# PhilipPragerUrbina/DOGERAY

Measured on AMD Instinct MI355X. Metric: Mrays/sec + ms/frame, 1M-tri .rts at 1920x1080, higher is better.
Workload: dtype f32

## Files before the change

### dogeray_amd/csrc/context.cpp

```cpp
#include <climits>
#include <exception>

#include "context.hpp"
#include "linearise.hpp"

using namespace dr;

namespace {

constexpr int ANY = INT_MIN;
struct Option { const char* name; int dr_context::*member; int lo, hi; unsigned only; bool reorders; };
const Option OPTIONS[] = {
    {"kernel", &dr_context::kernel, DR_KERNEL_TILE, DR_KERNEL_PERSISTENT, 0, false},
    {"occupancy", &dr_context::occupancy, 4, 6, 0, false},
    {"schedule", &dr_context::schedule, 0, 2, 0, false},
    {"heavy_factor", &dr_context::heavy_factor, -1, 1000, 0, true},
    {"coop_steps", &dr_context::coop_steps, 0, INT_MAX, 0, false},
    {"coop_lanes", &dr_context::coop_lanes, 1, 64, 0, false},
    {"split_parts", &dr_context::split_parts, 1, 8, 1u << 1 | 1u << 2 | 1u << 4 | 1u << 8, false},
    {"split_waves", &dr_context::split_waves, 1, 1000, 0, true},
    {"split_steps", &dr_context::split_steps, 16, 4080, 0, true},
    {"short_one_queue", &dr_context::short_one_queue, ANY, 0, 0, true},
    {"coop_rounds", &dr_context::coop_rounds, 1, 16, 0, false},
    {"reserve_cus", &dr_context::reserve_cus, 0, 64, 0, false},
    {"wave_log", &dr_context::wave_log_on, 0, 1, 0, false},
    {"coop_tiles_per_wave", &dr_context::coop_tiles_per_wave, 0, INT_MAX, 0, false},
    {"pipe_streams", &dr_context::pipe_streams, 2, dr_context::PIPE_STREAMS, 0, false},
    {"pipe_lean", &dr_context::pipe_lean, ANY, 0, 0, false},
    {"pipe_group", &dr_context::pipe_group, 1, dr_context::PIPE_GROUP_MAX, 0, false},
    {"xcd_regions", &dr_context::xcd_regions, ANY, 0, 0, true},
    {"batch_frames", &dr_context::batch_frames, 1, 256, 0, false},
    {"feedback", &dr_context::feedback, ANY, 0, 0, true},
    {"order_follows_camera", &dr_context::order_follows_camera, ANY, 0, 0, false},
    {"feedback_every", &dr_context::feedback_every, 1, INT_MAX, 0, false},
    {"wide_tree", &dr_context::wide_tree, 0, 2, 0, false},
    {"denoise_tiles", &dr_context::denoise_tiles, 0, 1, 0, false},
    {"moments", &dr_context::moments_opt, 0, 1, 0, false},
    {"denoise_variance", &dr_context::denoise_variance, 0, 1, 0, false},
    {"camera_cert", &dr_context::camera_cert, 0, 1, 0, false},
    {"cert_factor", &dr_context::cert_factor, 1, 10000, 0, false},
    {"cert_levels",  &dr_context::cert_levels, 0, 1, 0, false},
    {"camera_entry",  &dr_context::camera_entry, 0, 1, 0, false},
    {"sky_tiles",  &dr_context::sky_tiles, 0, 2, 0, false},
    {"trace_kernel",  &dr_context::trace_kernel, 0, 2, 0, false},
    {"radiance_kernel",  &dr_context::radiance_kernel, 0, 2, 0, false},
    {"allhits_kernel",  &dr_context::allhits_kernel, 0, 2, 0, false},
};

const Option* find_option(const std::string& name) {
  for (const Option& o : OPTIONS) if (name == o.name) return &o;
  return nullptr;
}

int flush_held(dr_context* c) {
  if (c->pipe_pending.empty()) return DR_OK;
  HIP_TRY(hipSetDevice(c->device));
  return pipeline_flush(c);
}

int set_option(dr_context* c, const std::string& name, int v) {
  const Option* o = find_option(name);
  if (!o) { set_error("unknown option '" + name + "'"); return DR_ERR_INVALID; }
  if (o->lo == ANY) v = v != 0;
  else if (v < o->lo || v > o->hi || (o->only && !(o->only >> v & 1u))) { set_error("value not supported for option '" + name + "'"); return DR_ERR_INVALID; }
  DR_TRY(flush_held(c));
  if (name == "split_steps") v &= ~15;
  else if (name == "wave_log") {
    if (v && !c->wave_log) {
      if (hipSetDevice(c->device) != hipSuccess || c->wave_log.alloc((size_t)WAVE_LOG_WAVES * 16) != DR_OK) { set_error("cannot allocate the wave log"); return DR_ERR_DEVICE; }
      (void)hipMemsetAsync(c->wave_log, 0, c->wave_log.n * sizeof(unsigned long long), c->stream);
    }
  }
  else if (name == "pipe_streams") {
    if (v != c->pipe_streams) {
      if (hipSetDevice(c->device) != hipSuccess || join_pipeline(c) != DR_OK || hipStreamSynchronize(c->stream) != hipSuccess) { set_error("pipe_streams: cannot drain the pipeline"); return DR_ERR_DEVICE; }
      for (int k = 0; k < dr_context::PIPE_DEPTH; k++) { c->pipe_slot[k].drained = true; c->pipe_slot[k].count = 0; c->pipe_slot[k].unwaited = 0; }
      c->pipe_parked.clear();
      c->pipe_next = 0; c->pipe_groups = 0;
    }
  }
  else if (name == "camera_cert" || name == "cert_factor" || o->member == &dr_context::cert_levels || o->member == &dr_context::camera_entry ||
           o->member == &dr_context::sky_tiles) c->cert_valid = false;
  c->*(o->member) = v;
  if (o->reorders) c->order_valid = false;
  return DR_OK;
}

}

dr_context::~dr_context() {
  (void)hipSetDevice(device);
  if (stream) (void)hipStreamSynchronize(stream);
  for (int k = 1; k < PIPE_STREAMS; k++) if (pipe_stream[k]) (void)hipStreamSynchronize(pipe_stream[k]);
  if (acc_stream) (void)hipStreamSynchronize(acc_stream);
  if (ev0) (void)hipEventDestroy(ev0);
  if (ev1) (void)hipEventDestroy(ev1);
  for (int k = 0; k < 2; k++) { if (pev0[k]) (void)hipEventDestroy(pev0[k]); if (pev1[k]) (void)hipEventDestroy(pev1[k]); }
  for (PipeSlot& sl : pipe_slot) {
    if (sl.rendered) (void)hipEventDestroy(sl.rendered);
// ... 298 lines not shown
```

### dogeray_amd/csrc/context.hpp

```cpp
#pragma once
#include <hip/hip_runtime_api.h>

#include <cmath>
#include <cstring>
#include <map>
#include <string>
#include <vector>

#include "kernels.hpp"
#include "params_host.hpp"
#include "scene_host.hpp"

#define HIP_TRY(expr)                                                                      \
  do {                                                                                     \
    hipError_t e_ = (expr);                                                                \
    if (e_ != hipSuccess) {                                                                \
      dr::set_error(std::string(#expr) + ": " + hipGetErrorString(e_));                    \
      return DR_ERR_DEVICE;                                                                \
    }                                                                                      \
  } while (0)

#define DR_TRY(expr)                                                                       \
  do {                                                                                     \
    const int rc_ = (expr);                                                                \
// ... 4 lines not shown

template <class T, bool PINNED = false>
struct DevMem {
  T* p = nullptr;
  size_t n = 0;
  DevMem() = default;
  DevMem(const DevMem&) = delete;
  DevMem& operator=(const DevMem&) = delete;
  ~DevMem() { release(); }
  operator T*() const { return p; }
  void release() {
    if (p) (void)(PINNED ? hipHostFree(p) : hipFree(p));
    p = nullptr; n = 0;
  }
  void swap(DevMem& o) { std::swap(p, o.p); std::swap(n, o.n); }
  int grow(size_t need, hipStream_t stream) {
    if (p && n >= need) return DR_OK;
    if (p) { HIP_TRY(hipStreamSynchronize(stream)); release(); }
    const hipError_t e = PINNED ? hipHostMalloc((void**)&p, need * sizeof(T), hipHostMallocDefault) : hipMalloc((void**)&p, need * sizeof(T));
    if (e != hipSuccess) { p = nullptr; set_error(std::string("cannot allocate ") + std::to_string(need * sizeof(T)) + " bytes: " + hipGetErrorString(e)); return DR_ERR_DEVICE; }
    n = need;
    return DR_OK;
  }
  int alloc(size_t count) { release(); return grow(count ? count : 1, nullptr); }
  int upload(const std::vector<T>& src) { DR_TRY(alloc(src.size())); return put(src.data(), src.size()); }
  int put(const T* src, size_t count) { if (count) HIP_TRY(hipMemcpy(p, src, count * sizeof(T), hipMemcpyHostToDevice)); return DR_OK; }
  int get(T* dst, size_t count) const { if (count) HIP_TRY(hipMemcpy(dst, p, count * sizeof(T), hipMemcpyDeviceToHost)); return DR_OK; }
};

struct GuideKey {
  bool valid = false;
  float st[13] = {0};
  int W = 0, H = 0;
  uint64_t gen = 0;
  bool matches(const float* settings13, int w, int h, uint64_t scene_gen) const {
    return valid && W == w && H == h && gen == scene_gen && memcmp(st, settings13, sizeof(st)) == 0;
  }
  void store(const float* settings13, int w, int h, uint64_t scene_gen) {
    memcpy(st, settings13, sizeof(st));
    W = w; H = h; gen = scene_gen; valid = true;
  }
};

struct LaunchSite {
  hipStream_t stream;
  bool hold_order;
  bool lean;
};

constexpr int TILE_COUNTERS = 1024;
constexpr int LAUNCH_COUNTERS = MAX_REGIONS + 1;

}

struct dr_context {
  template <class T> using DevMem = dr::DevMem<T>;
  int device = 0;
  hipStream_t stream = nullptr;
  hipEvent_t ev0 = nullptr, ev1 = nullptr;
  hipEvent_t pev0[2] = {nullptr, nullptr}, pev1[2] = {nullptr, nullptr};
  bool pending[2] = {false, false}; uint64_t pending_frames[2] = {0, 0}, pending_samples[2] = {0, 0}; int pending_next = 0;
  DevMem<dr::DevUnit> walk; size_t walk_bytes = 0;
  DevMem<dr::DevUnit> wide; size_t wide_bytes = 0; int wide_depth = 0, wide_nodes = 0; float wide_pmax = 0; dr::WideMu wide_mu = {0, 0, 0}; int wide_own_bounds = 0;
  int wide_tree = 2;
  DevMem<dr::DevPair> pairs;
  DevMem<dr::DevPrim> prims;
  DevMem<dr::DevShade> shade;
  DevMem<dr::DevTex> tex;
  DevMem<uint32_t> texels;
  int n_prims = 0, n_tex = 0, tree_depth = 0;
  std::vector<int> slot_to_orig;
  DevMem<int32_t> slot_to_orig_dev;
  DevMem<uint8_t> aov_staging;
  DevMem<uint8_t> query_staging;
  DevMem<uint32_t> query_scratch;
  DevMem<unsigned> query_cursor;
  int trace_kernel = 0, radiance_kernel = 0, allhits_kernel = 0;
  float near_lmax = 0;
  DevMem<float> dn_planes;
  dr::GuideKey dn_key;
  DevMem<uint8_t> dn_staging;
  DevMem<float> up_planes;
  dr::GuideKey up_key;
  int up_passes = 0;
  uint64_t scene_gen = 0;
  DevMem<int32_t> accum2;
  DevMem<int32_t> hist_buf[2];
  int32_t* hist = nullptr; int hist_cur = 0;
  DevMem<float> rp_planes[2];
  dr::GuideKey rp_key; int rp_cur = 0;
  DevMem<unsigned long long> rp_counts;
  int rp_passes = 0;
  int moments_opt = 0;
  int denoise_variance = 0;
  DevMem<unsigned long long> m2_buf[2];
  unsigned long long* m2 = nullptr; int m2_cur = 0;
  DevMem<unsigned long long> err_counts;
  DevMem<float> err_staging;
  int denoise_tiles = 1;
  int camera_cert = 1;
  int cert_factor = 40;
  int cert_levels = 1;
  DevMem<uint32_t> cert_mask;
  DevMem<uint32_t> cert_level;
  bool cert_valid = false;
  bool cert_ok = false;
  bool entry_ok = false;
  float cert_key[22] = {0};
  float cert_seen[22] = {0};
  float cert_k[dr::CERT_MAX_LEVELS + 1] = {1};
  int cert_tiles = 0;
  int camera_entry = 1;
  DevMem<uint32_t> wide_leaf_rec, wide_range;
  int wide_leaves = 0;
  DevMem<uint32_t> entry_mm;
  DevMem<uint32_t> cert_word;
  int sky_tiles = 2;
  DevMem<int> launch_order, launch_region_start, sky_list;
  DevMem<unsigned> sky_counts;
  bool sky_split_last = false;
  uint64_t cert_gen = 0;
  uint64_t order_gen = 0;
  uint64_t sky_key[5] = {0, 0, 0, 0, 0}; bool sky_key_valid = false;
  DevMem<int32_t> frame;
  DevMem<int32_t> accum; int accW = 0, accH = 0;
  DevMem<uint8_t> present;
  DevMem<int32_t> packed[2];
  DevMem<unsigned long long> counters;
  DevMem<unsigned> tile_counters; int tile_cursor = 0; int num_cus = 256;
  DevMem<unsigned> pixel_cost, tile_cost; DevMem<int> tile_order, region_start;
  int order_capacity = 0;
  bool order_valid = false;
  int order_age = 0;
  int order_follows_camera = 1;
  int feedback_every = 8;
  float order_key[18] = {0};
  int order_args[5] = {0, 0, 0, 0, 0};
  int feedback = 1;
  int stripe_mod = 1, stripe_rem = 0;
  int traversal = DR_TRAVERSAL_WIDE;
  int count = 0;
  int kernel = DR_KERNEL_PERSISTENT;
  int occupancy = 6;
  int schedule = 0;
  int xcd_regions = 1;
  int heavy_factor = 1;
  int coop_steps = 2;
  int coop_tiles_per_wave = 32;
  int coop_lanes = 8;
  int split_parts = 4;
  int split_waves = 12;
  int split_steps = 400;
  int short_one_queue = 1;
  int coop_rounds = 2;
  int reserve_cus = 0;
  int wave_log_on = 0;
  DevMem<unsigned long long> wave_log; int wave_log_waves = 0;
  int batch_frames = 32;
  float cur_settings[13] = {0};
  dr_stats stats;
  static constexpr int PIPE_STREAMS = 4;
  static constexpr int PIPE_DEPTH = PIPE_STREAMS + 1;
  int pipe_streams = 2;
  int pipe_lean = 0;
  hipStream_t pipe_stream[PIPE_STREAMS] = {nullptr, nullptr, nullptr, nullptr}, acc_stream = nullptr;
  static constexpr int PIPE_GROUP_MAX = 16;
  struct PipeSlot {
    DevMem<int32_t> frames; size_t elems_each = 0; int cap_frames = 0;
    int rect[6] = {-1, 0, 0, 0, 0, 0};
// ... 56 lines not shown
```

### dogeray_amd/csrc/context_render.cpp

```cpp
#include "context.hpp"

namespace dr {

void fill_scene(const dr_context* c, RenderParams& P) {
  P.walk = c->walk; P.walk_bytes = (uint32_t)c->walk_bytes; P.pairs = c->pairs; P.prims = c->prims; P.shade = c->shade; P.tex = c->tex; P.texels = c->texels;
  P.wide = c->wide; P.wide_bytes = (uint32_t)c->wide_bytes; P.wide_pmax = c->wide_pmax; P.wide_mu = c->wide_mu;
}

static int tiles_per_wave(const dr_context* c, const LaunchSite& site) {
  return site.lean ? 0 : c->coop_tiles_per_wave;
}

int make_params(dr_context* c, const LaunchSite& site, const float* st, int W, int H, float background, uint64_t seed, RenderParams& P, int batch_hint) {
  if (!c->walk) { set_error("no scene uploaded"); return DR_ERR_INVALID; }
  memset(&P, 0, sizeof(P));
  if (const char* why = fill_view_params(st, W, H, background, seed, c->stripe_mod, c->stripe_rem, P)) { set_error(why); return DR_ERR_INVALID; }
  if (P.backtex >= c->n_tex) { set_error("backtex refers to a texture that is not loaded"); return DR_ERR_INVALID; }
  memcpy(c->cur_settings, st, sizeof(c->cur_settings));
  fill_scene(c, P);
  P.counters = c->counters;
  P.wave_log = c->wave_log_on ? c->wave_log.p : nullptr;
  P.coop_steps = c->coop_steps; P.coop_rounds = c->coop_rounds; P.split_parts = c->split_parts;
  P.coop_lanes = c->coop_lanes;
  const int tiles = P.ncols * P.gy;
// ... 51 lines not shown
    c->cert_valid = false;
    c->cert_ok = c->entry_ok = false;
    c->cert_gen++;
    if (fill_cert_view(P, a_star, want_cert ? c->wide_mu.e : 1.0f, cv)) {
      if (c->cert_level.grow(cert_level_words(tiles), site.stream) != DR_OK || c->cert_word.grow((size_t)tiles, site.stream) != DR_OK ||
          (want_entry && c->entry_mm.grow(entry_mm_words(tiles), site.stream) != DR_OK)) return;
      for (float& k : c->cert_k) k = 1.0f;
      if (want_cert) {
        cert_ladder(c->cert_factor, c->cert_levels != 0, cv);
        if (c->cert_mask.grow(cert_mask_words(tiles, cv.n_levels), site.stream) != DR_OK) return;
        launch_cert_mask(site.stream, c->prims, c->n_prims, cv, c->cert_mask, c->cert_level, tiles);
        for (int g = 1; g <= CERT_MAX_LEVELS; g++) c->cert_k[g] = g <= cv.n_levels ? cert_factor_k(cv.level_a[g - 1]) : 1.0f;
      } else {
        (void)hipMemsetAsync(c->cert_level, 0, cert_level_words(tiles) * sizeof(uint32_t), site.stream);
      }
      launch_camera_entry(site.stream, c->wide, c->wide_leaf_rec, c->wide_range, c->wide_leaves, cv, want_entry ? c->entry_mm.p : nullptr, c->cert_level, c->cert_word, tiles);
      c->cert_ok = want_cert; c->entry_ok = want_entry;
    }
    memcpy(c->cert_key, key, sizeof(key));
    c->cert_tiles = tiles;
    c->cert_valid = true;
  }
  if (c->cert_ok || c->entry_ok) { P.cert_level = c->cert_word; memcpy(P.wide_cert_k, c->cert_k, sizeof(P.wide_cert_k)); }
}

bool sky_split(dr_context* c, const LaunchSite& site, RenderParams& P, int tiles, const int*& order, const int*& region_start, unsigned* pcost, unsigned* cursor) {
  if (!c->sky_tiles || !c->entry_ok || !P.cert_level || site.hold_order || site.stream != c->stream || P.out_frame_stride != 0) return false;
  if (P.max_depth <= 0 || !(P.spp_f > 0.0f)) return false;
  if (!plan_sky_split(plan_persistent(persistent_cfg(c, site), (long long)tiles * P.batch, P.coop_steps, false, P.wave_log != nullptr))) return false;
  const uint64_t key[5] = {c->cert_gen, order ? 1u : 0u, order ? c->order_gen : 0u, (uint64_t)tiles, (uint64_t)P.regions};
  const bool room = c->launch_order.n >= (size_t)tiles && c->sky_list.n >= (size_t)tiles && c->launch_region_start.p && c->sky_counts.p;
  if (!(room && c->sky_key_valid && memcmp(c->sky_key, key, sizeof(key)) == 0)) {
    c->sky_key_valid = false;
    if (c->launch_order.grow((size_t)tiles, site.stream) != DR_OK || c->sky_list.grow((size_t)tiles, site.stream) != DR_OK ||
        c->launch_region_start.grow(2 * MAX_REGIONS + 1, site.stream) != DR_OK || c->sky_counts.grow(2, site.stream) != DR_OK)
      return false;
    launch_sky_split(site.stream, order, region_start, P.region_start, P.cert_level, tiles, P.regions, c->launch_order, c->launch_region_start, c->sky_list, c->sky_counts);
    memcpy(c->sky_key, key, sizeof(key));
    c->sky_key_valid = true;
  }
  if (c->sky_tiles == 2) {
    P.sky_list = c->sky_list; P.sky_counts = c->sky_counts; P.sky_cursor = cursor;
    P.sky_chunk = sky_chunk_frames(P.batch, P.accumulate == 2 ? SKY_CHUNK : 0);
  } else launch_sky_tiles(site.stream, P, c->sky_list, c->sky_counts, pcost);
  order = c->launch_order; region_start = c->launch_region_start;
  return true;
}

}

int enqueue_frame(dr_context* c, const LaunchSite& site, const RenderParams& P_in) {
  RenderParams P = P_in;
  const int tiles = P.ncols * P.gy;
  if (uses_persistent(c)) {
    if (c->tile_cursor + LAUNCH_COUNTERS > TILE_COUNTERS) {
      (void)hipMemsetAsync(c->tile_counters, 0, TILE_COUNTERS * sizeof(unsigned), site.stream);
      c->tile_cursor = 0;
    }
    unsigned* counter = c->tile_counters + c->tile_cursor;
    c->tile_cursor += LAUNCH_COUNTERS;
    const int* order; unsigned* pcost;
    if (site.hold_order) {
      float geom[5];
      order_geometry(P, geom);
      order = (c->order_valid && c->order_capacity >= tiles && memcmp(c->order_key + 13, geom, sizeof(geom)) == 0) ? c->tile_order.p : nullptr;
      pcost = nullptr;
    } else feedback_buffers(c, site, P, tiles, order, pcost);
    if (!c->wave_log_on) P.wave_log = nullptr;
    cert_prepare(c, site, P, tiles);
    const int* launch_order = order; const int* launch_rstart = c->region_start;
    c->sky_split_last = sky_split(c, site, P, tiles, launch_order, launch_rstart, pcost, counter + MAX_REGIONS);
    const int log_waves = launch_persistent_kernel(site.stream, P, persistent_cfg(c, site), counter, launch_order, launch_rstart, pcost);
    if (log_waves < 0) { set_error("the persistent kernel has no build for this launch (launch_plan.hpp)"); return DR_ERR_DEVICE; }
    c->wave_log_waves = log_waves;
    if (pcost && !order) c->order_age = 0;
    if (pcost && (c->order_age < 2 || c->order_age % c->feedback_every == 0)) {
      const int split_limit = plan_split_limit(c->num_cus, c->occupancy, c->split_parts, c->split_waves);
      launch_tile_feedback(site.stream, c->pixel_cost, c->tile_cost, c->tile_order, c->region_start, tiles, P.regions, c->heavy_factor, c->split_steps, split_limit);
      c->order_gen++;
      c->order_args[0] = tiles; c->order_args[1] = P.regions; c->order_args[2] = c->heavy_factor; c->order_args[3] = c->split_steps; c->order_args[4] = split_limit;
      c->order_valid = true;
    }
    c->order_age++;
    return DR_OK;
  }
  c->sky_split_last = false;
  launch_tile_kernel(site.stream, P, traversal_of(c), c->count != 0, c->occupancy);
  return DR_OK;
}

}

using namespace dr;

namespace {

int launch_render(dr_context* c, const RenderParams& P) {
  int tiles = P.ncols * P.gy;
  if (tiles <= 0) return DR_OK;
  HIP_TRY(hipEventRecord(c->ev0, c->stream));
  DR_TRY(enqueue_frame(c, c->own_site(), P));
  HIP_TRY(hipGetLastError());
  HIP_TRY(hipEventRecord(c->ev1, c->stream));
  return DR_OK;
}

// ... 114 lines not shown
```

### dogeray_amd/csrc/device_layout.h

```cpp
#pragma once
#include <stdint.h>

namespace dr {

struct DevUnit {
  float f[4];
};
constexpr int WALK_UNITS_INTERNAL = 2;
constexpr int WALK_UNITS_LEAF = 4;
constexpr int WALK_SLOT_BITS = 26;
constexpr int WALK_KIND_SPHERE = 0, WALK_KIND_TRIANGLE = 1, WALK_KIND_NONE = 2;

inline uint32_t wide_node_first_child(const uint32_t* w) { return w[3] & 0xffffffu; }
inline uint32_t wide_node_valid(const uint32_t* w) { return (w[3] >> 24) & 15u; }
inline uint32_t wide_node_leaf_mask(const uint32_t* w) { return w[3] >> 28; }
inline uint32_t wide_node_lo(const uint32_t* w, int axis) { return w[4 + axis]; }
inline uint32_t wide_node_hi(const uint32_t* w, int axis) { return w[7 + axis]; }
inline uint32_t wide_node_scale24_bits(const uint32_t* w, int axis) { return axis == 0 ? w[10] << 16 : (axis == 1 ? w[10] & 0xffff0000u : w[11]); }
struct WideMu {
  float e;
  float l;
  float v;
};
struct CertView {
// ... 68 lines not shown
static_assert(CERT_MAX_LEVELS < (1 << ENTRY_SHIFT), "a grade fits under the entry code");
static_assert(sizeof(DevUnit) == 16, "DevUnit");
static_assert(sizeof(DevPair) == 64, "DevPair");
static_assert(sizeof(DevPrim) == 48, "DevPrim");
static_assert(sizeof(DevShade) == 128, "DevShade");
static_assert(sizeof(DevTex) == 16, "DevTex");

struct RenderParams {
  const DevUnit* walk;
  uint32_t walk_bytes;
  uint32_t pad_;
  const DevUnit* wide;
  uint32_t wide_bytes;
  float wide_pmax;
  const DevPair* pairs;
  const DevPrim* prims;
  const DevShade* shade;
  const DevTex* tex;
  const uint32_t* texels;
  int32_t* out;
  unsigned long long* counters;
  unsigned long long* wave_log;
  float from[3], llc[3], hor[3], ver[3], uu[3], vu[3];
  float lens_radius;
  float bgint;
  float scale;
  float spp_f;
  double den_w, den_h;
  uint64_t seed;
  int32_t W, H;
  int32_t gx, gy;
  int32_t ncols;
  int32_t stripe_mod, stripe_rem;
  uint32_t seed_stride;
  int32_t max_depth;
  int32_t backtex;
  int32_t accumulate;
  int32_t batch;
  uint64_t batch_seed_stride;
  int32_t coop_steps;
  int32_t coop_lanes;
  int32_t split_parts;
  int32_t coop_rounds;
  int32_t regions;
  uint32_t out_frame_stride;
  int32_t region_start[9];
  WideMu wide_mu;
  float wide_cert_k[CERT_MAX_LEVELS + 1];
  const uint32_t* cert_level;
  const int* sky_list;
  const unsigned* sky_counts;
  unsigned* sky_cursor;
  int32_t sky_chunk;
};

constexpr int DN_MISS = -1;
constexpr int DN_OUTSIDE = -2147483647 - 1;
constexpr int DN_MAX_ITERATIONS = 10;
constexpr int DN_MAX_NORMAL_POWER_LOG2 = 16;
struct DnParams {
  int iterations;
  float sigma_luminance;
  int normal_power_log2;
  float sigma_depth;
  int demodulate;
  int material_stop;
};

constexpr int UP_BLOCK = 0, UP_GUIDED = 1;
struct UpParams {
  int mode;
  int normal_power_log2;
  float sigma_depth;
  int demodulate;
  int material_stop;
};

constexpr int RP_VALID = 0, RP_MASKED = 1, RP_OFFSCREEN = 2, RP_REJECTED = 3;
constexpr int RP_MAX_HISTORY = 65535;
struct RpParams {
  int max_history;
  float normal_cos;
  float plane_tolerance;
  uint32_t material_mask;
  int sky;
};
struct RpCamera {
  float from[3], llc[3], hor[3], ver[3];
  double den_w, den_h;
};
struct RpProj {
  double L[3];
  double cN[3];
  double hor[3], ver[3];
  double LcN;
  double hh, vv;
};

constexpr long long MO_CAP = 1ll << 26;
constexpr int MO_BINS = 16;
constexpr int MO_WORDS = 3 + MO_BINS;
constexpr int MO_ESTIMATED = 0, MO_ABOVE = 1, MO_SUM_VAR = 2, MO_BIN0 = 3;

}
```

### dogeray_amd/csrc/device_shade.hpp

```cpp
#pragma once
#include "device_rng.hpp"
#include "device_surface.hpp"

namespace dr {

struct Path { V3 rayo, raydir, atten; };

struct ShadeCtx { V3 hitpoint, N, ocolor; float add_x, rough, ir, r5; int mat; bool front; };
__device__ __forceinline__ bool shade_needs_sphere(const ShadeCtx& sc) { return sc.mat == 0 || sc.mat == 3 || sc.mat == 5; }

template <bool COUNT>
__device__ __forceinline__ bool shade_material(const RenderParams& P, const Path& path, V3 hitpoint, V3 N, V3 texco, float4 s4, float4 s5, float4 s6, Xorwow& rng, Ctr& c,
                                               ShadeCtx& sc, V3& emitted) {
  const V3 raydir = path.raydir;
  bool front = dot(raydir, N) < 0;
  N = front ? N : N * splat(-1.0f);
  V3 col = mk(s4.z, s4.w, s5.x);
  float add_x = s5.y, rough = s5.z;
  int mat = __float_as_int(s5.w), texnum = __float_as_int(s6.x), rtexnum = __float_as_int(s6.y);
  int flags = __float_as_int(s6.z);
  V3 ocolor = col;
  if (texnum >= 0) {
    ocolor = rgb_of(tex_fetch<COUNT>(P.tex, P.texels, texnum, texco.x, -texco.y + 1, c));
  } else if (flags & 2) {
// ... 113 lines not shown
    V3 colr = rgb_of(tex_fetch<COUNT>(P.tex, P.texels, P.backtex, tt.x, -tt.y + 1, c));
    return atten * colr * splat(P.bgint);
  }
  float t2 = (float)(0.5 * ((double)u.y + 1.0));
  float omt = (float)(1.0 - (double)t2);
  V3 sky = splat(omt) * mk(1.0f, 1.0f, 1.0f) + splat(t2) * mk(0.5f, 0.7f, 1.0f);
  return atten * sky * splat(P.bgint);
}

template <bool COUNT, class Closest>
__device__ __forceinline__ V3 trace_path(const RenderParams& P, const Closest& closest, V3 origin, V3 dir, Xorwow& rng, Ctr& c) {
  Path path; path.rayo = origin; path.raydir = dir; path.atten = splat(1.0f);
  for (int i = 0; i < P.max_depth; i++) {
    Hit h = closest(path.rayo, path.raydir, c);
    if (h.t > 0.0f) {
      V3 emitted;
      if (!shade_hit<COUNT>(P, path, h.t, h.slot, rng, c, emitted)) return emitted;
    } else {
      return shade_miss<COUNT>(P, path, c);
    }
  }
  return mk(0, 0, 0);
}

__device__ __forceinline__ void camera_prepare(const RenderParams& P, int x, int y, Xorwow& rng, float& nu, float& nv) {
  nu = (float)(((double)(float)x + rng.uniform_double()) / P.den_w);
  nv = (float)(((double)(float)y + rng.uniform_double()) / P.den_h);
}
__device__ __forceinline__ void camera_finish(const RenderParams& P, float nu, float nv, V3 disk, V3& origin, V3& dir) {
  V3 from = ld3(P.from), llc = ld3(P.llc), hor = ld3(P.hor), ver = ld3(P.ver), uu = ld3(P.uu), vu = ld3(P.vu);
  V3 rd = splat(P.lens_radius) * disk;
  V3 offset = uu * splat(rd.x) + vu * splat(rd.y);
  dir = llc + splat(nu) * hor + splat(nv) * ver - from - offset;
  origin = from + offset;
}
__device__ __forceinline__ void camera_ray(const RenderParams& P, int x, int y, Xorwow& rng, V3& origin, V3& dir) {
  float nu, nv;
  camera_prepare(P, x, y, rng, nu, nv);
  camera_finish(P, nu, nv, rand_in_unit_disk(rng), origin, dir);
}
__device__ __forceinline__ uint64_t sample_seed(const RenderParams& P, int x, int y, int s, int frame = 0) {
  return P.seed + (uint64_t)frame * P.batch_seed_stride + (uint64_t)s * 0x9E3779B97F4A7C15ull +
         (uint64_t)((uint32_t)x + (uint32_t)y * P.seed_stride);
}
__device__ __forceinline__ void store_pixel(const RenderParams& P, int x, int y, V3 color, size_t frame_offset = 0) {
  int r = f2i(color.x * 255 * P.scale), g = f2i(color.y * 255 * P.scale), b = f2i(color.z * 255 * P.scale);
  int32_t* px = P.out + frame_offset + ((size_t)x * (size_t)P.H + (size_t)y) * 3;
  if (P.accumulate == 2) {
    atomicAdd(px + 0, r); atomicAdd(px + 1, g); atomicAdd(px + 2, b);
  } else if (P.accumulate) { px[0] += r; px[1] += g; px[2] += b; }
  else { px[0] = r; px[1] = g; px[2] = b; }
}

template <bool COUNT, class Closest>
__device__ __forceinline__ void render_pixel(const RenderParams& P, const Closest& closest, int x, int y, Ctr& c, bool* camera_ray_next = nullptr ) {
  V3 color = mk(0, 0, 0);
  for (int s = 0; (float)s < P.spp_f; ++s) {
    Xorwow rng;
    rng.init(sample_seed(P, x, y, s));
    if (COUNT) c.samples++;
    V3 origin, dir;
    camera_ray(P, x, y, rng, origin, dir);
    if (camera_ray_next) *camera_ray_next = true;
    color = color + trace_path<COUNT>(P, closest, origin, dir, rng, c);
  }
  store_pixel(P, x, y, color);
}

}
```

### dogeray_amd/csrc/kernels_render.hip

```cpp
#include <hip/hip_runtime.h>

#include "device_core.hpp"
#include "device_coop.hpp"
#include "device_sky.hpp"
#include "kernels.hpp"
#include "../../include/dogeray_amd.h"

namespace dr {

template <bool COUNT, int MODE, int OCC>
__global__ __launch_bounds__(256, OCC) void render_kernel(RenderParams P) {
  __shared__ int lds_stack[MODE == DR_TRAVERSAL_ORDERED ? ORDERED_STACK * 256 : (MODE == DR_TRAVERSAL_WIDE ? WIDE_STACK * 256 : 1)];
  const int wave = threadIdx.x >> 6, lane = threadIdx.x & 63;
  const int tile = blockIdx.x * 4 + wave;
  Ctr c = {0, 0, 0, 0, 0, 0, 0, 0};
  if (tile < P.ncols * P.gy) {
    const int col = tile / P.gy, by = tile - col * P.gy;
    const int bx = P.stripe_rem + col * P.stripe_mod;
    const int x = bx * 8 + (lane >> 3), y = by * 8 + (lane & 7);
    if (MODE == DR_TRAVERSAL_ORDERED) {
      int* stack = lds_stack + wave * (ORDERED_STACK * 64) + lane;
      auto closest = [&](V3 o, V3 d, Ctr& cc) { return closest_hit_ordered<COUNT>(P.pairs, P.prims, o, d, cc, stack); };
      render_pixel<COUNT>(P, closest, x, y, c);
    } else if (MODE == DR_TRAVERSAL_WIDE) {
// ... 156 lines not shown
        asm volatile("" ::: "memory");
      }
      DR_MARK("phase_shade");
      bool ended = false;
      V3 radiance = mk(0, 0, 0);
      ShadeCtx sc; sc.hitpoint = sc.N = sc.ocolor = mk(0, 0, 0); sc.add_x = sc.rough = sc.ir = sc.r5 = 0.0f; sc.mat = -1; sc.front = false;
      bool scatter_me = false;
      if (shade_me) {
        if (tr.best_slot >= 0 && tr.best_t > 0.0f) {
          if (UV_CARRIED || FETCH_LAZY ? !shade_prepare_hit<UV_CARRIED, FETCH_LAZY>(P, path, tr.best_t, tr.best_slot, hit_u, hit_v, rng, c, sc, radiance)
                                       : !shade_prepare<COUNT>(P, path, tr.best_t, tr.best_slot, rng, c, sc, radiance)) ended = true;
          else {
            if (BOUNCE_HOME) bounce = __float_as_int(st[WS_BOUNCE * 64]);
            bounce++;
            if (bounce >= P.max_depth) ended = true;
            else scatter_me = true;
            if (BOUNCE_HOME) st[WS_BOUNCE * 64] = __int_as_float(bounce);
          }
        } else {
          radiance = shade_miss<COUNT>(P, path, c);
          ended = true;
        }
      }
      DR_MARK("phase_unstash");
      if (WIDE) {
        asm volatile("" ::: "memory");
        color = mk(st[WS_COLOR_X * 64], st[WS_COLOR_Y * 64], st[WS_COLOR_Z * 64]);
        { const int xy = __float_as_int(st[WS_XY * 64]); px = (int)((unsigned)xy >> 16) - 1; py = xy & 0xffff; }
        pcode = __float_as_int(st[WS_PCODE * 64]);
        frame = (int)((unsigned)__float_as_int(st[WS_W1 * 64]) >> (16 * WS_W1_FRAME_HALF)); sample = __float_as_int(st[WS_SAMPLE * 64]);
        steps = __float_as_uint(st[WS_STEPS * 64]);
        if (UV_CARRIED) { st[WS_STEPS * 64] = hit_v; st[WS_COLOR_X * 64] = hit_u; }
        if (COOP) rstart = __float_as_uint(st[WS_RSTART * 64]);
      } else {
        asm volatile("" ::: "memory");
        color = mk(st[TS_COLOR_X * 64], st[TS_COLOR_Y * 64], st[TS_COLOR_Z * 64]);
        px = __float_as_int(st[TS_PX * 64]); py = __float_as_int(st[TS_PY * 64]); pcode = __float_as_int(st[TS_PCODE * 64]);
        frame = __float_as_int(st[TS_FRAME * 64]); sample = __float_as_int(st[TS_SAMPLE * 64]);
        steps = __float_as_uint(st[TS_STEPS * 64]); rstart = __float_as_uint(st[TS_RSTART * 64]);
      }
      if (shade_me) {
        if (ended) {
          color = color + radiance;
          sample++;
          tr.node = LANE_REFILL;
        } else {
          trav_begin(tr);
          rstart = steps;
          fresh_ray = true;
          if (COUNT) c.rays++;
        }
      }
      bool want_pixel = false;
      if (tr.node == LANE_REFILL) {
        if (px >= 0 && (float)sample < P.spp_f && !degenerate) {
        } else {
          if (px >= 0) {
            store_pixel(P, px, py, color, PERFRAME ? (size_t)frame * (size_t)P.out_frame_stride : (size_t)0);
            if (pixel_cost) pixel_cost[pcode & PCODE_MASK] = steps;
          }
          px = -1;
          want_pixel = true;
        }
      }
      if (WIDE && COOP && splitting) {
        held = __ballot(px >= 0 && pcode < 0) != 0ull;
        if (!held && tr.node == LANE_RETIRED && share < 0 && !(cur_tile >= ntiles && regions_left == 0)) { tr.node = LANE_REFILL; want_pixel = true; }
      }
      unsigned long long need = __ballot(want_pixel);
      unsigned cam_cert = 0u;
      while (need != 0ull) {
        if (cur_next >= cur_limit) {
          if (WIDE && COOP && held) {
            if (want_pixel) { tr.node = LANE_RETIRED; want_pixel = false; }
            break;
          }
          cur_tile = ntiles;
          cur_next = 0; cur_limit = 64; cur_split = false;
          while (regions_left > 0) {
            const int r0 = region_start ? region_start[region] : P.region_start[region];
            const int r1 = region_start ? region_start[region + 1] : P.region_start[region + 1];
            unsigned t = 0;
            if (lane == 0) t = atomicAdd(tile_counter + region, 1u);
            const int q = (int)__builtin_amdgcn_readfirstlane(t);
            const int nsplit = splitting ? region_start[MAX_REGIONS + 1 + region] : 0;
            if (q < (r1 - r0 + nsplit * (P.split_parts - 1)) * P.batch) {
              int tt = q / P.batch;
              cur_frame = q - tt * P.batch;
              if (WIDE && COOP && tt < nsplit * P.split_parts) {
                const int part = tt % P.split_parts, width = 64 / P.split_parts;
                tt /= P.split_parts;
                cur_next = part * width; cur_limit = cur_next + width; cur_split = true; held = true;
              } else {
                tt -= nsplit * (P.split_parts - 1);
              }
              cur_tile = tile_order ? tile_order[r0 + tt] : r0 + tt;
              if (BOUNCE_HOME) cur_cert = P.cert_level != nullptr ? P.cert_level[cur_tile] : 0u;
              break;
            }
            region = region + 1 == P.regions ? 0 : region + 1;
            regions_left--;
          }
        }
        if (cur_tile >= ntiles) {
          if (want_pixel) { tr.node = LANE_RETIRED; want_pixel = false; }
          if (WAVE_LOG && r_empty == 0ull) r_empty = __builtin_amdgcn_s_memrealtime();
          break;
        }
        const int rank = (int)__builtin_amdgcn_mbcnt_hi((unsigned)(need >> 32), __builtin_amdgcn_mbcnt_lo((unsigned)need, 0u));
        const int avail = cur_limit - cur_next;
        if (want_pixel && rank < avail) {
          const int l = cur_next + rank;
          const int col = cur_tile / P.gy, by = cur_tile - col * P.gy;
          px = (P.stripe_rem + col * P.stripe_mod) * 8 + (l >> 3);
          py = by * 8 + (l & 7);
          pcode = (cur_tile * 64 + l) | (cur_split ? PCODE_SPLIT : 0);
          frame = cur_frame;
          steps = 0;
          sample = 0;
          color = mk(0, 0, 0);
          want_pixel = false;
          cam_cert = cur_cert;
        }
        const int n = __popcll(need);
        cur_next += n < avail ? n : avail;
        need = __ballot(want_pixel);
      }
      DR_MARK("phase_camera");
      bool new_path = false;
      float cam_nu = 0.0f, cam_nv = 0.0f;
      if (tr.node == LANE_REFILL && px >= 0) {
        if (degenerate) {
          sample = 0x7fffffff;
          if (COUNT) c.samples++;
        } else {
          rng.init(sample_seed(P, px, py, sample, frame));
          if (COUNT) { c.samples++; c.rays++; }
          camera_prepare(P, px, py, rng, cam_nu, cam_nv);
          new_path = true;
        }
      }
      {
        unsigned my_turns = 0;
        const int draw_kind = scatter_me && shade_needs_sphere(sc) ? 3 : (new_path ? 2 : 0);
        const V3 pt = rand_points_merged<COUNT>(rng, draw_kind, &my_turns);
        if (COUNT) {
          unsigned wave_turns = my_turns;
          for (int off = 32; off > 0; off >>= 1) { const unsigned o = (unsigned)__shfl_xor((int)wave_turns, off, 64); wave_turns = o > wave_turns ? o : wave_turns; }
          unsigned long long lane_turns = my_turns;
          for (int off = 32; off > 0; off >>= 1) lane_turns += __shfl_xor(lane_turns, off, 64);
          const unsigned n_sphere = (unsigned)__popcll(__ballot(draw_kind == 3)), n_disk = (unsigned)__popcll(__ballot(draw_kind == 2));
          const unsigned n_retired = (unsigned)__popcll(__ballot(tr.node == LANE_RETIRED));
          if (lane == 0) atomicAdd(&P.counters[STAT_TURN_HIST + (wave_turns < (unsigned)(STAT_TURN_BINS - 1) ? wave_turns : (unsigned)(STAT_TURN_BINS - 1))], 1ull);
          pb_cands += lane_turns; pb_turns += wave_turns; pb_sphere += n_sphere; pb_disk += n_disk; pb_retired += n_retired;
        }
        if (scatter_me) shade_scatter(path, sc, pt, rng);
        if (new_path) {
          camera_finish(P, cam_nu, cam_nv, pt, path.rayo, path.raydir);
          path.atten = splat(1.0f);
          bounce = 0;
          if (BOUNCE_HOME) st[WS_BOUNCE * 64] = __int_as_float(0);
          trav_begin(tr);
          if (BOUNCE_HOME) tr.node = (int)cam_cert >> ENTRY_SHIFT;
          rstart = steps;
          fresh_ray = true;
        }
      }
      if (BOUNCE_HOME && fresh_ray) reinterpret_cast<unsigned char*>(st + WS_W1 * 64)[WS_W1_GRADE_BYTE] = (unsigned char)(new_path ? cam_cert & ((1u << ENTRY_SHIFT) - 1u) : 0u);
      if (COUNT && ray_log && fresh_ray && frame == 0) {
        atomicAdd(&P.counters[STAT_LOG_RAYS], 1ull);
// ... 238 lines not shown
```

### dogeray_amd/csrc/launch_plan.hpp

```cpp
#pragma once
#include "../../include/dogeray_amd.h"
#include "device_layout.h"

namespace dr {

constexpr int MAX_REGIONS = 8;
constexpr int WAVE_LOG_WAVES = 16384;

struct PersistentCfg {
  int traversal;
  int occupancy;
  int schedule;
  int num_cus;
  int coop_tiles_per_wave;
  bool count;
};

struct PersistentBuild { int count, occ, trav_min, park_min, unroll, wide, coop, perframe; };
inline bool operator==(const PersistentBuild& a, const PersistentBuild& b) {
  return a.count == b.count && a.occ == b.occ && a.trav_min == b.trav_min && a.park_min == b.park_min && a.unroll == b.unroll && a.wide == b.wide &&
         a.coop == b.coop && a.perframe == b.perframe;
}

#define DR_SCHEDULE_0 32, 20, 2, 12, 4
// ... 23 lines not shown
  bool clear_wave_log;
};

inline bool short_launch(long long work, int tiles_per_wave, long long waves) { return work < (long long)tiles_per_wave * waves; }

inline bool persistent_can_store_per_frame(const PersistentCfg& cfg) {
  return cfg.traversal == DR_TRAVERSAL_WIDE && !cfg.count && cfg.schedule == 0 && cfg.occupancy >= 6;
}

inline PersistentPlan plan_persistent(const PersistentCfg& cfg, long long work, int coop_steps, bool per_frame, bool wave_log_on) {
  const PersistentSchedule& s = PERSISTENT_SCHEDULES[cfg.schedule == 0 ? 0 : cfg.schedule == 1 ? 1 : 2];
  const bool wide = cfg.traversal == DR_TRAVERSAL_WIDE, six = persistent_can_store_per_frame(cfg);
  per_frame = per_frame && six;
  auto blocks_for = [&](int occ) {
    const int blocks = cfg.num_cus * occ;
    return (long long)blocks * 4 > work ? (int)((work + 3) / 4) : blocks;
  };
  PersistentPlan p;
  if (six && !(coop_steps > 0 && short_launch(work, cfg.coop_tiles_per_wave, (long long)cfg.num_cus * 5 * 4))) {
    p.build = {false, 6, s.trav_min, s.park_min, s.unroll, true, false, per_frame};
    p.blocks = blocks_for(6);
    p.log_waves = 0; p.clear_wave_log = true;
    return p;
  }
  const int occ = cfg.occupancy >= 5 ? 5 : 4;
  p.blocks = blocks_for(occ);
  p.clear_wave_log = wave_log_on && p.blocks * 4 > WAVE_LOG_WAVES;
  p.log_waves = wave_log_on && !p.clear_wave_log ? p.blocks * 4 : 0;
  const bool coop = per_frame || (coop_steps > 0 && short_launch(work, cfg.coop_tiles_per_wave, (long long)p.blocks * 4));
  if (!wide) p.build = {cfg.count, occ, s.trav_min, s.park_min, s.unroll, false, true, false};
  else if (cfg.count) p.build = {true, occ, s.trav_min, s.park_min, s.unroll, true, false, false};
  else if (coop) p.build = {false, occ, s.trav_min, s.coop_park, s.coop_unroll, true, true, per_frame};
  else p.build = {false, occ, s.trav_min, s.park_min, s.unroll, true, false, false};
  if (wide && !coop) p.log_waves = 0;
  return p;
}

inline bool plan_sky_split(const PersistentPlan& p) { return p.build.wide && !p.build.count && !p.build.coop && !p.build.perframe; }

#ifndef DR_SKY_CHUNK
#define DR_SKY_CHUNK 0
#endif
constexpr int SKY_CHUNK = DR_SKY_CHUNK;
struct SkyUnit { int index, first, count; };
constexpr int sky_chunk_frames(int batch, int chunk) { return chunk > 0 && chunk < batch ? chunk : (batch > 0 ? batch : 1); }
constexpr int sky_chunks(int batch, int chunk) { return batch > 0 ? (batch + sky_chunk_frames(batch, chunk) - 1) / sky_chunk_frames(batch, chunk) : 0; }
constexpr unsigned sky_units(unsigned n_sky, int batch, int chunk) { return n_sky * (unsigned)sky_chunks(batch, chunk); }
constexpr SkyUnit sky_unit(unsigned u, int batch, int chunk) {
  const unsigned chunks = (unsigned)sky_chunks(batch, chunk), index = u / chunks;
  const int frames = sky_chunk_frames(batch, chunk), first = (int)(u - index * chunks) * frames;
  return SkyUnit{(int)index, first, batch - first < frames ? batch - first : frames};
}

inline int plan_regions(int tiles, int batch_hint, bool xcd_regions, bool short_one_queue, int tiles_per_wave, int num_cus) {
  int regions = xcd_regions ? MAX_REGIONS : 1;
  if (tiles < 64 * MAX_REGIONS) regions = 1;
  if (short_one_queue && short_launch((long long)tiles * batch_hint, tiles_per_wave, (long long)num_cus * 5 * 4)) regions = 1;
  return regions;
}

inline int plan_split_limit(int num_cus, int occupancy, int split_parts, int split_waves) {
  return split_parts > 1 ? (int)((long long)num_cus * (occupancy >= 5 ? 5 : 4) * 4 * split_waves / (100 * split_parts)) : 0;
}

enum { QUERY_KERNEL_PLAIN = 0, QUERY_KERNEL_PERSISTENT = 1 };
enum { QUERY_FORCE_NONE = 0, QUERY_FORCE_PLAIN = 1, QUERY_FORCE_PERSISTENT = 2 };
struct RayListPlan { int kernel, blocks; };
inline RayListPlan plan_ray_list(long long n, bool can_persist, int force, long long min_rays, int occ, int chunk, int num_cus) {
  const bool persistent = can_persist && (force == QUERY_FORCE_PERSISTENT || (force != QUERY_FORCE_PLAIN && n >= min_rays));
  if (!persistent) return {QUERY_KERNEL_PLAIN, (int)((n + 255) / 256)};
  const long long full = (long long)num_cus * occ, need = (n + 4 * chunk - 1) / (4 * chunk);
  return {QUERY_KERNEL_PERSISTENT, (int)(need < full ? need : full)};
}

constexpr int TRACE_OCC = 6, TRACE_REFILL_MIN = 8, TRACE_PARK = 20;
constexpr int TRACE_CHUNK = 128;
constexpr long long TRACE_PERSISTENT_MIN_RAYS = 1 << 25;
struct TracePlan {
  int kernel;
  int traversal;
  int blocks;
};
inline TracePlan plan_trace(long long n, int traversal, bool has_wide, int num_cus, int force) {
  const int walk = (traversal == DR_TRAVERSAL_WIDE && !has_wide) ? DR_TRAVERSAL_THREADED : traversal;
  const RayListPlan l = plan_ray_list(n, walk == DR_TRAVERSAL_WIDE, force, TRACE_PERSISTENT_MIN_RAYS, TRACE_OCC, TRACE_CHUNK, num_cus);
  return {l.kernel, walk, l.blocks};
}

constexpr int RADIANCE_OCC = 5, RADIANCE_REFILL_MIN = 32, RADIANCE_PARK = 20;
constexpr int RADIANCE_CHUNK = 64;
constexpr long long RADIANCE_PERSISTENT_MIN_RAYS = 1 << 22;
struct RadiancePlan {
  int kernel;
  int traversal;
  int blocks;
};
inline RadiancePlan plan_radiance(long long n, int traversal, bool has_wide, int num_cus, int force) {
  const int walk = (traversal == DR_TRAVERSAL_WIDE && !has_wide) ? DR_TRAVERSAL_THREADED : traversal;
  const RayListPlan l = plan_ray_list(n, walk == DR_TRAVERSAL_WIDE, force, RADIANCE_PERSISTENT_MIN_RAYS, RADIANCE_OCC, RADIANCE_CHUNK, num_cus);
  return {l.kernel, walk, l.blocks};
}

struct NearestPlan {
  bool wide;
  int blocks;
};
// ... 27 lines not shown
```

### dogeray_amd/csrc/params_host.hpp

```cpp
#pragma once
#include <cmath>
#include <cstdint>
#include <cstring>
#include <string>

#include "../../include/dogeray_amd.h"
#include "device_layout.h"

namespace dr {

struct V3h { float x, y, z; };
inline V3h hsub(V3h a, V3h b) { return {a.x - b.x, a.y - b.y, a.z - b.z}; }
inline V3h hmul(V3h a, V3h b) { return {a.x * b.x, a.y * b.y, a.z * b.z}; }
inline V3h hdiv(V3h a, V3h b) { return {a.x / b.x, a.y / b.y, a.z / b.z}; }
inline V3h hsplat(float a) { return {a, a, a}; }
inline float hdot(V3h a, V3h b) { return a.x * b.x + a.y * b.y + a.z * b.z; }
inline V3h hcross(V3h a, V3h b) { return {a.y * b.z - a.z * b.y, a.z * b.x - a.x * b.z, a.x * b.y - a.y * b.x}; }
inline V3h hnorm(V3h v) { float inv = 1.0f / sqrtf(hdot(v, v)); return {v.x * inv, v.y * inv, v.z * inv}; }
inline void st3(float* d, V3h v) { d[0] = v.x; d[1] = v.y; d[2] = v.z; }
inline int hf2i(float f) {
  if (f != f) return 0;
  if (f >= 2147483648.0f) return 2147483647;
  if (f <= -2147483648.0f) return (-2147483647 - 1);
  return (int)f;
}

inline const char* fill_view_params(const float* st, int W, int H, float background, uint64_t seed, int stripe_mod, int stripe_rem, RenderParams& P) {
  if (W <= 0 || H <= 0 || W > 65000 || H > 65000 || (size_t)W * (size_t)H > (size_t)1 << 28) return "bad frame size";
  const int div = hf2i(st[11]);
  if (div < 1) return "divisor must be >= 1";
  float aspect = float(W / st[11]) / float(H / st[11]);
  float fov = (float)((double)st[8] * M_PI / 180);
  float vh = (float)(2.0 * (double)tanf(fov / 2));
  float vw = aspect * vh;
  V3h from = {st[0], st[1], st[2]}, at = {st[3], st[4], st[5]};
  float focus = st[7];
  V3h vup = {0, 1, 0};
  V3h wu = hnorm(hsub(from, at));
  V3h uu = hnorm(hcross(vup, wu));
  V3h vu = hcross(wu, uu);
  V3h hor = hmul(hmul(hsplat(focus), hsplat(vw)), uu);
  V3h ver = hmul(hmul(hsplat(focus), hsplat(vh)), vu);
  V3h llc = hsub(hsub(hsub(from, hdiv(hor, hsplat(2))), hdiv(ver, hsplat(2))), hmul(hsplat(focus), wu));
  st3(P.from, from); st3(P.llc, llc); st3(P.hor, hor); st3(P.ver, ver); st3(P.uu, uu); st3(P.vu, vu);
  P.lens_radius = st[6] / 2;
  P.bgint = background;
  P.spp_f = st[10];
  P.scale = (float)(1.0 / (double)st[10]);
  P.den_w = (double)float(W / st[11]);
  P.den_h = (double)float(H / st[11]);
  P.seed = seed;
  P.W = W; P.H = H;
  P.gx = W / div / 8; P.gy = H / div / 8;
  P.stripe_mod = stripe_mod; P.stripe_rem = stripe_rem;
  P.ncols = P.gx > stripe_rem ? (P.gx - stripe_rem + stripe_mod - 1) / stripe_mod : 0;
  P.seed_stride = 8u * (unsigned)P.gx;
  P.max_depth = hf2i(st[9]);
  P.backtex = hf2i(st[12]);
  P.batch = 1;
  P.batch_seed_stride = 0;
  return nullptr;
}

inline bool fill_cert_view(const RenderParams& P, double a_star, float e_own, CertView& cv) {
  memset(&cv, 0, sizeof(cv));
  if (!(e_own > 0.0f) || !(a_star >= 1e-4)) return false;
  double hor[3], ver[3], uu[3], vu[3];
  for (int a = 0; a < 3; a++) { cv.from[a] = P.from[a]; cv.llc[a] = P.llc[a]; hor[a] = P.hor[a]; ver[a] = P.ver[a]; uu[a] = P.uu[a]; vu[a] = P.vu[a]; }
  auto dot = [](const double* a, const double* b) { return a[0] * b[0] + a[1] * b[1] + a[2] * b[2]; };
  auto norm = [&](const double* a) { return std::sqrt(dot(a, a)); };
  double w[3] = {hor[1] * ver[2] - hor[2] * ver[1], hor[2] * ver[0] - hor[0] * ver[2], hor[0] * ver[1] - hor[1] * ver[0]};
  const double wn = norm(w);
  if (!(wn > 0) || !std::isfinite(wn)) return false;
  double lf[3] = {cv.llc[0] - cv.from[0], cv.llc[1] - cv.from[1], cv.llc[2] - cv.from[2]};
  for (int a = 0; a < 3; a++) w[a] /= wn;
  if (dot(lf, w) < 0) for (int a = 0; a < 3; a++) w[a] = -w[a];
  memcpy(cv.w, w, sizeof(w));
  cv.D = dot(lf, w);
  const double hh = dot(hor, hor), hv = dot(hor, ver), vv = dot(ver, ver), det = hh * vv - hv * hv;
  if (!(det > 0)) return false;
  for (int a = 0; a < 3; a++) { cv.du[a] = (vv * hor[a] - hv * ver[a]) / det; cv.dv[a] = (hh * ver[a] - hv * hor[a]) / det; }
  cv.du_n = norm(cv.du); cv.dv_n = norm(cv.dv);
  const double r = std::fabs((double)P.lens_radius), fn = norm(cv.from);
  cv.r_o = 1.001 * r * (norm(uu) + norm(vu)) + 0x1p-22 * (fn + 2.0 * r) + 1e-30;
  cv.eps_d = 0x1p-20 * (norm(cv.llc) + norm(hor) + norm(ver) + fn + cv.r_o);
  cv.dmin = cv.D - cv.r_o - 1e-9 * (norm(hor) + norm(ver)) - cv.eps_d;
  cv.den_w = P.den_w; cv.den_h = P.den_h;
  cv.a_star = a_star;
  cv.level_a[0] = a_star; cv.n_levels = 1; cv.base = 0;
  cv.e_own = (double)e_own * (1.0 + 1e-6);
  cv.nx = 8 * P.gx; cv.ny = 8 * P.gy; cv.gy = P.gy;
  cv.stripe_mod = P.stripe_mod; cv.stripe_rem = P.stripe_rem; cv.ncols = P.ncols;
  const double all[] = {cv.D, cv.r_o, cv.eps_d, cv.dmin, cv.du_n, cv.dv_n, fn};
  for (double v : all) if (!std::isfinite(v)) return false;
  return cv.dmin > 8.0 * cv.r_o && cv.dmin > 0;
}

inline void fill_reproject_camera(const RenderParams& P, RpCamera& C) {
  for (int a = 0; a < 3; a++) { C.from[a] = P.from[a]; C.llc[a] = P.llc[a]; C.hor[a] = P.hor[a]; C.ver[a] = P.ver[a]; }
  C.den_w = P.den_w; C.den_h = P.den_h;
}
inline bool fill_reproject_proj(const RpCamera& C, RpProj& J) {
  auto dot = [](const double* a, const double* b) { return (a[0] * b[0] + a[1] * b[1]) + a[2] * b[2]; };
  for (int a = 0; a < 3; a++) { J.L[a] = (double)C.llc[a] - (double)C.from[a]; J.hor[a] = (double)C.hor[a]; J.ver[a] = (double)C.ver[a]; }
  J.cN[0] = J.hor[1] * J.ver[2] - J.hor[2] * J.ver[1];
  J.cN[1] = J.hor[2] * J.ver[0] - J.hor[0] * J.ver[2];
  J.cN[2] = J.hor[0] * J.ver[1] - J.hor[1] * J.ver[0];
  if (dot(J.cN, J.L) < 0) for (int a = 0; a < 3; a++) J.cN[a] = -J.cN[a];
  J.LcN = dot(J.L, J.cN);
  J.hh = dot(J.hor, J.hor); J.vv = dot(J.ver, J.ver);
  return std::isfinite(J.LcN) && J.LcN != 0.0;
}
constexpr DnParams DN_DEFAULTS = {5, 4.0f, 7, 1.0f, 1, 1};
// ... 53 lines not shown
```

Before: 9409.

## Interleave batched frames per pixel and merge same-pixel atomic stores within a wave

Adds a sample_order option, on by default, that reorders how batched-frame samples are handed to lanes: consecutive work indices now walk the frames of one pixel before moving to the next pixel, using a magic-number division. In batched accumulate mode this puts several lanes of a wave on the same output pixel, so a new merged store path combines their colours (through LDS slots by default, or a DPP wave reduction) and issues one set of global atomics per pixel. The aim is to cut global atomic contention and traffic on the accumulation buffer. The cost is extra LDS work and branching per store, and a different ray coherence pattern.

New measurement: 9717 (median of 6 runs). 1.03x the previous value.

```diff
diff --git a/dogeray_amd/csrc/context.cpp b/dogeray_amd/csrc/context.cpp
--- a/dogeray_amd/csrc/context.cpp
+++ b/dogeray_amd/csrc/context.cpp
@@ -45,6 +45,7 @@
     {"trace_kernel",  &dr_context::trace_kernel, 0, 2, 0, false},
     {"radiance_kernel",  &dr_context::radiance_kernel, 0, 2, 0, false},
     {"allhits_kernel",  &dr_context::allhits_kernel, 0, 2, 0, false},
+    {"sample_order",  &dr_context::sample_order, 0, 1, 0, false},
 };
 
 const Option* find_option(const std::string& name) {
diff --git a/dogeray_amd/csrc/context.hpp b/dogeray_amd/csrc/context.hpp
--- a/dogeray_amd/csrc/context.hpp
+++ b/dogeray_amd/csrc/context.hpp
@@ -80,6 +80,10 @@
 constexpr int LAUNCH_COUNTERS = MAX_REGIONS + 1;
 
 }
+
+#ifndef DR_SAMPLE_ORDER
+#define DR_SAMPLE_ORDER 1
+#endif
 
 struct dr_context {
   template <class T> using DevMem = dr::DevMem<T>;
@@ -143,6 +147,7 @@
   int wide_leaves = 0;
   DevMem<uint32_t> entry_mm;
   DevMem<uint32_t> cert_word;
+  int sample_order = DR_SAMPLE_ORDER;
   int sky_tiles = 2;
   DevMem<int> launch_order, launch_region_start, sky_list;
   DevMem<unsigned> sky_counts;
diff --git a/dogeray_amd/csrc/context_render.cpp b/dogeray_amd/csrc/context_render.cpp
--- a/dogeray_amd/csrc/context_render.cpp
+++ b/dogeray_amd/csrc/context_render.cpp
@@ -127,6 +127,7 @@
 int enqueue_frame(dr_context* c, const LaunchSite& site, const RenderParams& P_in) {
   RenderParams P = P_in;
   const int tiles = P.ncols * P.gy;
+  P.sample_magic = sample_order_magic(c->sample_order, P.batch);
   if (uses_persistent(c)) {
     if (c->tile_cursor + LAUNCH_COUNTERS > TILE_COUNTERS) {
       (void)hipMemsetAsync(c->tile_counters, 0, TILE_COUNTERS * sizeof(unsigned), site.stream);
diff --git a/dogeray_amd/csrc/device_layout.h b/dogeray_amd/csrc/device_layout.h
--- a/dogeray_amd/csrc/device_layout.h
+++ b/dogeray_amd/csrc/device_layout.h
@@ -144,6 +144,7 @@
   const unsigned* sky_counts;
   unsigned* sky_cursor;
   int32_t sky_chunk;
+  uint32_t sample_magic;
 };
 
 constexpr int DN_MISS = -1;
diff --git a/dogeray_amd/csrc/device_shade.hpp b/dogeray_amd/csrc/device_shade.hpp
--- a/dogeray_amd/csrc/device_shade.hpp
+++ b/dogeray_amd/csrc/device_shade.hpp
@@ -189,6 +189,55 @@
   else { px[0] = r; px[1] = g; px[2] = b; }
 }
 
+#ifndef DR_HOST_BUILD
+#ifndef DR_STORES_MERGED
+#define DR_STORES_MERGED 2
+#endif
+constexpr int STORES_MERGED = DR_STORES_MERGED;
+__device__ __forceinline__ int wave_sum(int v) {
+  v += __builtin_amdgcn_update_dpp(0, v, 0x111, 0xf, 0xf, true);
+  v += __builtin_amdgcn_update_dpp(0, v, 0x112, 0xf, 0xf, true);
+  v += __builtin_amdgcn_update_dpp(0, v, 0x114, 0xf, 0xf, true);
+  v += __builtin_amdgcn_update_dpp(0, v, 0x118, 0xf, 0xf, true);
+  v += __builtin_amdgcn_update_dpp(0, v, 0x142, 0xa, 0xf, true);
+  v += __builtin_amdgcn_update_dpp(0, v, 0x143, 0xc, 0xf, true);
+  return __builtin_amdgcn_readlane(v, 63);
+}
+__device__ __forceinline__ void store_pixels_merged(const RenderParams& P, bool store_me, int key, int x, int y, V3 color) {
+  const int r = f2i(color.x * 255 * P.scale), g = f2i(color.y * 255 * P.scale), b = f2i(color.z * 255 * P.scale);
+  unsigned long long todo = __ballot(store_me);
+  while (todo != 0ull) {
+    const int lead = __builtin_ctzll(todo);
+    const bool mine = store_me && key == __builtin_amdgcn_readlane(key, lead);
+    const int sr = wave_sum(mine ? r : 0), sg = wave_sum(mine ? g : 0), sb = wave_sum(mine ? b : 0);
+    if ((int)(threadIdx.x & 63) == lead) {
+      int32_t* px = P.out + ((size_t)x * (size_t)P.H + (size_t)y) * 3;
+      atomicAdd(px + 0, sr); atomicAdd(px + 1, sg); atomicAdd(px + 2, sb);
+    }
+    todo &= ~__ballot(mine);
+  }
+}
+__device__ __forceinline__ void store_pixels_merged_lds(const RenderParams& P, int* ws, int lane, bool store_me, int key, int x, int y, V3 color) {
+  if (!store_me) return;
+  int* const slot = ws + ((key & 63) - lane);
+  slot[0] = key; slot[2 * 64] = 0; slot[3 * 64] = 0; slot[4 * 64] = 0;
+  asm volatile("" ::: "memory");
+  const bool ok = slot[0] == key;
+  if (ok) {
+    slot[1 * 64] = lane;
+    atomicAdd(slot + 2 * 64, f2i(color.x * 255 * P.scale)); atomicAdd(slot + 3 * 64, f2i(color.y * 255 * P.scale)); atomicAdd(slot + 4 * 64, f2i(color.z * 255 * P.scale));
+  }
+  asm volatile("" ::: "memory");
+  int r, g, b;
+  if (ok) {
+    if (slot[1 * 64] != lane) return;
+    r = slot[2 * 64]; g = slot[3 * 64]; b = slot[4 * 64];
+  } else { r = f2i(color.x * 255 * P.scale); g = f2i(color.y * 255 * P.scale); b = f2i(color.z * 255 * P.scale); }
+  int32_t* px = P.out + ((size_t)x * (size_t)P.H + (size_t)y) * 3;
+  atomicAdd(px + 0, r); atomicAdd(px + 1, g); atomicAdd(px + 2, b);
+}
+#endif
+
 template <bool COUNT, class Closest>
 __device__ __forceinline__ void render_pixel(const RenderParams& P, const Closest& closest, int x, int y, Ctr& c, bool* camera_ray_next = nullptr ) {
   V3 color = mk(0, 0, 0);
diff --git a/dogeray_amd/csrc/kernels_render.hip b/dogeray_amd/csrc/kernels_render.hip
--- a/dogeray_amd/csrc/kernels_render.hip
+++ b/dogeray_amd/csrc/kernels_render.hip
@@ -232,11 +232,18 @@
         }
       }
       bool want_pixel = false;
+      static_assert(WS_SAMPLE - WS_COLOR_Y == 4, "five consecutive stash words");
+      const bool merged = STORES_MERGED != 0 && WIDE && !PERFRAME && P.sample_magic != 0u && P.accumulate == 2;
+      if (merged) {
+        const bool store_me = tr.node == LANE_REFILL && px >= 0 && !((float)sample < P.spp_f && !degenerate);
+        if (STORES_MERGED == 2) store_pixels_merged_lds(P, reinterpret_cast<int*>(st) + WS_COLOR_Y * 64, lane, store_me, pcode, px, py, color);
+        else store_pixels_merged(P, store_me, pcode, px, py, color);
+      }
       if (tr.node == LANE_REFILL) {
         if (px >= 0 && (float)sample < P.spp_f && !degenerate) {
         } else {
           if (px >= 0) {
-            store_pixel(P, px, py, color, PERFRAME ? (size_t)frame * (size_t)P.out_frame_stride : (size_t)0);
+            if (!merged) store_pixel(P, px, py, color, PERFRAME ? (size_t)frame * (size_t)P.out_frame_stride : (size_t)0);
             if (pixel_cost) pixel_cost[pcode & PCODE_MASK] = steps;
           }
           px = -1;
@@ -290,12 +297,12 @@
         const int rank = (int)__builtin_amdgcn_mbcnt_hi((unsigned)(need >> 32), __builtin_amdgcn_mbcnt_lo((unsigned)need, 0u));
         const int avail = cur_limit - cur_next;
         if (want_pixel && rank < avail) {
-          const int l = cur_next + rank;
+          const TileSample ts = tile_sample(P.sample_magic, P.batch, cur_frame * 64 + cur_next + rank);
           const int col = cur_tile / P.gy, by = cur_tile - col * P.gy;
-          px = (P.stripe_rem + col * P.stripe_mod) * 8 + (l >> 3);
-          py = by * 8 + (l & 7);
-          pcode = (cur_tile * 64 + l) | (cur_split ? PCODE_SPLIT : 0);
-          frame = cur_frame;
+          px = (P.stripe_rem + col * P.stripe_mod) * 8 + (ts.p >> 3);
+          py = by * 8 + (ts.p & 7);
+          pcode = (cur_tile * 64 + ts.p) | (cur_split ? PCODE_SPLIT : 0);
+          frame = ts.f;
           steps = 0;
           sample = 0;
           color = mk(0, 0, 0);
diff --git a/dogeray_amd/csrc/launch_plan.hpp b/dogeray_amd/csrc/launch_plan.hpp
--- a/dogeray_amd/csrc/launch_plan.hpp
+++ b/dogeray_amd/csrc/launch_plan.hpp
@@ -99,6 +99,17 @@
   return SkyUnit{(int)index, first, batch - first < frames ? batch - first : frames};
 }
 
+constexpr int SAMPLE_ORDER_MAX_BATCH = 256;
+struct TileSample { int p, f; };
+constexpr uint32_t sample_order_magic(int order, int batch) {
+  return order == 1 && batch > 1 && batch <= SAMPLE_ORDER_MAX_BATCH ? (uint32_t)((0x100000000ull + (uint64_t)batch - 1ull) / (uint64_t)batch) : 0u;
+}
+constexpr TileSample tile_sample(uint32_t magic, int batch, int j) {
+  if (magic == 0u) return TileSample{j & 63, j >> 6};
+  const int p = (int)(uint32_t)(((uint64_t)(uint32_t)j * (uint64_t)magic) >> 32);
+  return TileSample{p, j - p * batch};
+}
+
 inline int plan_regions(int tiles, int batch_hint, bool xcd_regions, bool short_one_queue, int tiles_per_wave, int num_cus) {
   int regions = xcd_regions ? MAX_REGIONS : 1;
   if (tiles < 64 * MAX_REGIONS) regions = 1;
diff --git a/dogeray_amd/csrc/params_host.hpp b/dogeray_amd/csrc/params_host.hpp
--- a/dogeray_amd/csrc/params_host.hpp
+++ b/dogeray_amd/csrc/params_host.hpp
@@ -59,6 +59,7 @@
   P.backtex = hf2i(st[12]);
   P.batch = 1;
   P.batch_seed_stride = 0;
+  P.sample_magic = 0;
   return nullptr;
 }
 
```
